# IRVLUTD/handnet-pipeline

Hardware: AMD Instinct MI355X
Metric: end-to-end frames/sec (FCOS+A2J, 640x480) (higher is better)
Workload: dtype f16x3 (fp32 values split into fp16 hi+lo, 3 MFMAs, fp32 accumulate; fp32 I/O); 1 GPU; Full HandNet pipeline (FCOS -> crop -> A2J), 640x480 RGB-D (BASELINE config 4); batch_per_gpu=32, global_batch=32, frame=640x480 RGB-D, parallelism=frames sharded over 1 GPU(s), one all-gather of per-frame records per step, rccl_ranks=1, ipc_mode=HSA_ENABLE_IPC_MODE_LEGACY=0, hipgraph=False

## Files before the change

handnet-pipeline_amd/csrc/conv_stem_direct.hip:

```cpp
#include "hn_common.h"

namespace {

typedef float f32x4 __attribute__((ext_vector_type(4)));
typedef _Float16 f16x8 __attribute__((ext_vector_type(8)));
typedef __attribute__((address_space(3))) void lds_void;
typedef __attribute__((address_space(1))) const void gbl_void;

constexpr int kPR = 15, kPC = 17;
constexpr int kQR = 7, kQC = 8;
constexpr int kIR = 2 * (kPR - 1) + 7;
constexpr int kIP = (2 * (kPC - 1) + 8) / 2;
constexpr int kPlanePieces = kIR * kIP;
constexpr int kPatchPieces = ((2 * kPlanePieces + 255) / 256) * 256;
constexpr int kWPieces = 64 * 7 * 8;
constexpr int kCout = 64;
constexpr int kPitch = kCout + 4;

struct StemParams {
  const _Float16* x;
  const _Float16* w;
  const float* bias;
  _Float16* y;
  int n, hb, wb, oh, ow, poh, pow_, ty, tx;
  long plane;
  int terms;
  int* range_flag;
};

__global__ __launch_bounds__(256, 2) void conv_stem_pool_direct_kernel(const StemParams p) {
  extern __shared__ __attribute__((aligned(1024))) char smem[];
  _Float16* patch = reinterpret_cast<_Float16*>(smem);
  _Float16* wbank = reinterpret_cast<_Float16*>(smem + kPatchPieces * 16);
  const int tid = threadIdx.x, lane = tid & 63, wave = tid >> 6, lg = lane >> 4, px = lane & 15;
  int lid;
  {
    const int bid = blockIdx.x, nb = gridDim.x;
    const int q = nb >> 3, rr = nb & 7, xcd = bid & 7, loc = bid >> 3;
    lid = (xcd < rr ? xcd * (q + 1) : rr * (q + 1) + (xcd - rr) * q) + loc;
  }
  const int per_img = p.ty * p.tx;
  const int img = lid / per_img;
  const int rem = lid - img * per_img;
  const int pty = rem / p.tx, ptx = rem - pty * p.tx;
  const int oy0 = 2 * kQR * pty - 1, ox0 = 2 * kQC * ptx - 1;
  const int r0 = 2 * oy0, c0p = ox0;

  const int wave_base = __builtin_amdgcn_readfirstlane(wave) * 64;
#pragma unroll
  for (int rnd = 0; rnd < kPatchPieces / 256; ++rnd) {
    const int q = rnd * 256 + tid;
    int pl = q >= kPlanePieces ? 1 : 0;
    int k = q - pl * kPlanePieces;
    if (k >= kPlanePieces) { pl = 1; k = kPlanePieces - 1; }
    const int row = k / kIP, pc = k - row * kIP;
    int sr = r0 + row, sc = c0p + pc;
    sr = sr < 0 ? 0 : (sr < p.hb ? sr : p.hb - 1);
    sc = sc < 0 ? 0 : (sc < (p.wb >> 1) ? sc : (p.wb >> 1) - 1);
    const _Float16* src = p.x + pl * p.plane + (((long)img * p.hb + sr) * p.wb + sc * 2) * 4;
    __builtin_amdgcn_global_load_lds((gbl_void*)src, (lds_void*)(smem + (rnd * 256 + wave_base) * 16), 16, 0, 0);
  }
#pragma unroll
  for (int rnd = 0; rnd < kWPieces / 256; ++rnd) {
    const _Float16* src = p.w + (long)(rnd * 256 + tid) * 8;
    __builtin_amdgcn_global_load_lds((gbl_void*)src, (lds_void*)(reinterpret_cast<char*>(wbank) + (rnd * 256 + wave_base) * 16), 16, 0,
                                     0);
  }

  int a_off[4];
  bool ok[4];
#pragma unroll
  for (int i = 0; i < 4; ++i) {
    int row = wave * 64 + i * 16 + px;
    ok[i] = row < kPR * kPC;
    row = ok[i] ? row : kPR * kPC - 1;
    const int pr = row / kPC, pc = row - pr * kPC;
    const int oy = oy0 + pr, ox = ox0 + pc;
    ok[i] = ok[i] && (unsigned)oy < (unsigned)p.oh && (unsigned)ox < (unsigned)p.ow;
    a_off[i] = ((2 * pr) * kIP + pc + lg) * 16;
  }
  const int b_off = (px * 7) * 128 + lg * 16;

  f32x4 acc[4][4];
#pragma unroll
  for (int i = 0; i < 4; ++i)
#pragma unroll
    for (int j = 0; j < 4; ++j) acc[i][j] = f32x4{0.f, 0.f, 0.f, 0.f};

  asm volatile("s_waitcnt vmcnt(0)" ::: "memory");
  __syncthreads();

  const char* pa = reinterpret_cast<const char*>(patch);
  const char* pb = reinterpret_cast<const char*>(wbank);
#pragma unroll 1
  for (int ky = 0; ky < 7; ++ky) {
    f16x8 ah[4], al[4], bh[4], bl[4];
#pragma unroll
    for (int i = 0; i < 4; ++i) {
      ah[i] = *reinterpret_cast<const f16x8*>(pa + a_off[i] + ky * (kIP * 16));
      al[i] = *reinterpret_cast<const f16x8*>(pa + a_off[i] + ky * (kIP * 16) + kPlanePieces * 16);
    }
#pragma unroll
    for (int j = 0; j < 4; ++j) {
      bh[j] = *reinterpret_cast<const f16x8*>(pb + b_off + j * (16 * 7 * 128) + ky * 128);
      bl[j] = *reinterpret_cast<const f16x8*>(pb + b_off + j * (16 * 7 * 128) + ky * 128 + 64);
    }
    if (p.terms == 3) {
#pragma unroll
      for (int i = 0; i < 4; ++i)
#pragma unroll
        for (int j = 0; j < 4; ++j) acc[i][j] = __builtin_amdgcn_mfma_f32_16x16x32_f16(bh[j], al[i], acc[i][j], 0, 0, 0);
#pragma unroll
      for (int i = 0; i < 4; ++i)
#pragma unroll
        for (int j = 0; j < 4; ++j) acc[i][j] = __builtin_amdgcn_mfma_f32_16x16x32_f16(bl[j], ah[i], acc[i][j], 0, 0, 0);
    }
#pragma unroll
    for (int i = 0; i < 4; ++i)
#pragma unroll
      for (int j = 0; j < 4; ++j) acc[i][j] = __builtin_amdgcn_mfma_f32_16x16x32_f16(bh[j], ah[i], acc[i][j], 0, 0, 0);
  }

  __syncthreads();
  float* fp = reinterpret_cast<float*>(smem);
  const int nsub = (lg & 1) * 16 + (lg >> 1) * 8;
#pragma unroll
  for (int i = 0; i < 4; ++i) {
    const int row = wave * 64 + i * 16 + px;
#pragma unroll
    for (int jp = 0; jp < 2; ++jp) {
      f32x4 x = acc[i][2 * jp], y = acc[i][2 * jp + 1];
#pragma unroll
      for (int r = 0; r < 4; ++r) {
        const auto s = __builtin_amdgcn_permlane16_swap(__float_as_uint(x[r]), __float_as_uint(y[r]), false, false);
        x[r] = __uint_as_float(s[0]);
        y[r] = __uint_as_float(s[1]);
      }
      const int n = jp * 32 + nsub;
      const f32x4 b0 = *reinterpret_cast<const f32x4*>(p.bias + n), b1 = *reinterpret_cast<const f32x4*>(p.bias + n + 4);
#pragma unroll
      for (int e = 0; e < 4; ++e) {
        x[e] = ok[i] ? hn::relu(x[e] + b0[e]) : 0.f;
        y[e] = ok[i] ? hn::relu(y[e] + b1[e]) : 0.f;
      }
      *reinterpret_cast<f32x4*>(fp + row * kPitch + n) = x;
      *reinterpret_cast<f32x4*>(fp + row * kPitch + n + 4) = y;
    }
  }
  __syncthreads();
  for (int item = tid; item < kQR * kQC * (kCout / 8); item += 256) {
    const int c8 = item & (kCout / 8 - 1), pp = item / (kCout / 8);
    const int pr = pp / kQC, pc = pp - pr * kQC;
    const int gy = kQR * pty + pr, gx = kQC * ptx + pc;
    if (gy >= p.poh || gx >= p.pow_) continue;
    f32x4 m0 = {0.f, 0.f, 0.f, 0.f}, m1 = m0;
#pragma unroll
    for (int dy = 0; dy < 3; ++dy)
#pragma unroll
      for (int dx = 0; dx < 3; ++dx) {
        const float* src = fp + ((2 * pr + dy) * kPC + 2 * pc + dx) * kPitch + c8 * 8;
        const f32x4 a = *reinterpret_cast<const f32x4*>(src), b = *reinterpret_cast<const f32x4*>(src + 4);
#pragma unroll
        for (int e = 0; e < 4; ++e) {
          m0[e] = hn::max_nan(m0[e], a[e]);
          m1[e] = hn::max_nan(m1[e], b[e]);
        }
      }
    f16x8 hi, lo;
    if (p.range_flag) {
      float mg = 0.f;
#pragma unroll
      for (int e = 0; e < 4; ++e) mg = hn::max_nan(mg, hn::range_mag(m0[e], m1[e]));
      if (!(mg <= 65504.f)) *p.range_flag = 1;
    }
#pragma unroll
    for (int e = 0; e < 4; ++e) {
      const _Float16 h0 = (_Float16)m0[e], h1 = (_Float16)m1[e];
      hi[e] = h0;
      hi[4 + e] = h1;
      lo[e] = (_Float16)(m0[e] - (float)h0);
      lo[4 + e] = (_Float16)(m1[e] - (float)h1);
    }
    _Float16* dst = p.y + (((long)img * p.poh + gy) * p.pow_ + gx) * (2 * kCout) + (c8 >> 2) * 64 + (c8 & 3) * 8;
    *reinterpret_cast<f16x8*>(dst) = hi;
    *reinterpret_cast<f16x8*>(dst + 32) = lo;
  }
}

}

namespace hn {

int stem_pool_direct(const void* x16, int n, int ph, int pw, const void* w16, const float* bias, void* y, int terms, hipStream_t st) {
  const int hb = ph + 6, wb = pw + 6;
  StemParams p;
  p.x = (const _Float16*)x16; p.w = (const _Float16*)w16; p.bias = bias; p.y = (_Float16*)y;
  p.n = n; p.hb = hb; p.wb = wb;
  p.oh = (hb - 7) / 2 + 1; p.ow = (wb - 7) / 2 + 1;
  p.poh = (p.oh + 2 - 3) / 2 + 1; p.pow_ = (p.ow + 2 - 3) / 2 + 1;
  p.ty = hn::cdiv(p.poh, kQR); p.tx = hn::cdiv(p.pow_, kQC);
  p.plane = (long)n * hb * wb * 4;
  p.terms = terms == 1 ? 1 : 3;
  p.range_flag = hn::range_flag_ptr();
  HN_CHECK_ARG(wb % 2 == 0 && (uintptr_t)x16 % 16 == 0 && (uintptr_t)w16 % 16 == 0 && (uintptr_t)y % 16 == 0 &&
                   (uintptr_t)bias % 16 == 0, "stem image rows / tensors must be 16-byte aligned");
  HN_CHECK_ARG((int64_t)n * p.ty * p.tx < (int64_t)1 << 31, "too many patches");
  constexpr int LDS_BYTES = kPatchPieces * 16 + kWPieces * 16;
  static_assert(LDS_BYTES <= 80 * 1024 && 256 * kPitch * 4 <= LDS_BYTES, "two workgroups per CU; the pooling patch reuses the space");
  static bool attr_set[64] = {};
  int dev = 0;
  HN_CHECK_HIP(hipGetDevice(&dev));
  if (dev < 0 || dev >= 64 || !attr_set[dev]) {
    HN_CHECK_HIP(hipFuncSetAttribute((const void*)conv_stem_pool_direct_kernel, hipFuncAttributeMaxDynamicSharedMemorySize, LDS_BYTES));
    if (dev >= 0 && dev < 64) attr_set[dev] = true;
  }
  hipLaunchKernelGGL(conv_stem_pool_direct_kernel, dim3(n * p.ty * p.tx), dim3(256), LDS_BYTES, st, p);
  HN_CHECK_LAUNCH("conv_stem_pool_direct_kernel");
  return HN_OK;
}

}
```

Measured before the change: 1167 frames/s.

## Make stem conv persistent and pool per 16-channel column tile

After: 1169 frames/s (median of 4 runs). About the same (+0.1%).

```diff
diff --git a/handnet-pipeline_amd/csrc/conv_stem_direct.hip b/handnet-pipeline_amd/csrc/conv_stem_direct.hip
--- a/handnet-pipeline_amd/csrc/conv_stem_direct.hip
+++ b/handnet-pipeline_amd/csrc/conv_stem_direct.hip
@@ -4,6 +4,7 @@
 
 typedef float f32x4 __attribute__((ext_vector_type(4)));
 typedef _Float16 f16x8 __attribute__((ext_vector_type(8)));
+typedef _Float16 f16x4 __attribute__((ext_vector_type(4)));
 typedef __attribute__((address_space(3))) void lds_void;
 typedef __attribute__((address_space(1))) const void gbl_void;
 
@@ -15,7 +16,7 @@
 constexpr int kPatchPieces = ((2 * kPlanePieces + 255) / 256) * 256;
 constexpr int kWPieces = 64 * 7 * 8;
 constexpr int kCout = 64;
-constexpr int kPitch = kCout + 4;
+constexpr int kPitch = 16 + 4;
 
 struct StemParams {
   const _Float16* x;
@@ -28,162 +29,153 @@
   int* range_flag;
 };
 
+__device__ __forceinline__ int xcd_remap(int v, int total) {
+  const int q = total >> 3, rr = total & 7, xcd = v & 7, loc = v >> 3;
+  return (xcd < rr ? xcd * (q + 1) : rr * (q + 1) + (xcd - rr) * q) + loc;
+}
+
 __global__ __launch_bounds__(256, 2) void conv_stem_pool_direct_kernel(const StemParams p) {
   extern __shared__ __attribute__((aligned(1024))) char smem[];
   _Float16* patch = reinterpret_cast<_Float16*>(smem);
   _Float16* wbank = reinterpret_cast<_Float16*>(smem + kPatchPieces * 16);
   const int tid = threadIdx.x, lane = tid & 63, wave = tid >> 6, lg = lane >> 4, px = lane & 15;
-  int lid;
-  {
-    const int bid = blockIdx.x, nb = gridDim.x;
-    const int q = nb >> 3, rr = nb & 7, xcd = bid & 7, loc = bid >> 3;
-    lid = (xcd < rr ? xcd * (q + 1) : rr * (q + 1) + (xcd - rr) * q) + loc;
-  }
   const int per_img = p.ty * p.tx;
-  const int img = lid / per_img;
-  const int rem = lid - img * per_img;
-  const int pty = rem / p.tx, ptx = rem - pty * p.tx;
-  const int oy0 = 2 * kQR * pty - 1, ox0 = 2 * kQC * ptx - 1;
-  const int r0 = 2 * oy0, c0p = ox0;
-
+  const int total = p.n * per_img;
   const int wave_base = __builtin_amdgcn_readfirstlane(wave) * 64;
-#pragma unroll
-  for (int rnd = 0; rnd < kPatchPieces / 256; ++rnd) {
-    const int q = rnd * 256 + tid;
-    int pl = q >= kPlanePieces ? 1 : 0;
-    int k = q - pl * kPlanePieces;
-    if (k >= kPlanePieces) { pl = 1; k = kPlanePieces - 1; }
-    const int row = k / kIP, pc = k - row * kIP;
-    int sr = r0 + row, sc = c0p + pc;
-    sr = sr < 0 ? 0 : (sr < p.hb ? sr : p.hb - 1);
-    sc = sc < 0 ? 0 : (sc < (p.wb >> 1) ? sc : (p.wb >> 1) - 1);
-    const _Float16* src = p.x + pl * p.plane + (((long)img * p.hb + sr) * p.wb + sc * 2) * 4;
-    __builtin_amdgcn_global_load_lds((gbl_void*)src, (lds_void*)(smem + (rnd * 256 + wave_base) * 16), 16, 0, 0);
-  }
+
 #pragma unroll
   for (int rnd = 0; rnd < kWPieces / 256; ++rnd) {
     const _Float16* src = p.w + (long)(rnd * 256 + tid) * 8;
     __builtin_amdgcn_global_load_lds((gbl_void*)src, (lds_void*)(reinterpret_cast<char*>(wbank) + (rnd * 256 + wave_base) * 16), 16, 0,
                                      0);
   }
-
-  int a_off[4];
-  bool ok[4];
-#pragma unroll
-  for (int i = 0; i < 4; ++i) {
-    int row = wave * 64 + i * 16 + px;
-    ok[i] = row < kPR * kPC;
-    row = ok[i] ? row : kPR * kPC - 1;
-    const int pr = row / kPC, pc = row - pr * kPC;
-    const int oy = oy0 + pr, ox = ox0 + pc;
-    ok[i] = ok[i] && (unsigned)oy < (unsigned)p.oh && (unsigned)ox < (unsigned)p.ow;
-    a_off[i] = ((2 * pr) * kIP + pc + lg) * 16;
-  }
   const int b_off = (px * 7) * 128 + lg * 16;
-
-  f32x4 acc[4][4];
-#pragma unroll
-  for (int i = 0; i < 4; ++i)
-#pragma unroll
-    for (int j = 0; j < 4; ++j) acc[i][j] = f32x4{0.f, 0.f, 0.f, 0.f};
-
-  asm volatile("s_waitcnt vmcnt(0)" ::: "memory");
-  __syncthreads();
-
-  const char* pa = reinterpret_cast<const char*>(patch);
-  const char* pb = reinterpret_cast<const char*>(wbank);
+  f32x4 bj[4];
+#pragma unroll
+  for (int j = 0; j < 4; ++j) bj[j] = *reinterpret_cast<const f32x4*>(p.bias + 16 * j + 4 * lg);
+
 #pragma unroll 1
-  for (int ky = 0; ky < 7; ++ky) {
-    f16x8 ah[4], al[4], bh[4], bl[4];
+  for (int v = blockIdx.x; v < total; v += gridDim.x) {
+    const int lid = xcd_remap(v, total);
+    const int img = lid / per_img;
+    const int rem = lid - img * per_img;
+    const int pty = rem / p.tx, ptx = rem - pty * p.tx;
+    const int oy0 = 2 * kQR * pty - 1, ox0 = 2 * kQC * ptx - 1;
+    const int r0 = 2 * oy0, c0p = ox0;
+
+#pragma unroll
+    for (int rnd = 0; rnd < kPatchPieces / 256; ++rnd) {
+      const int q = rnd * 256 + tid;
+      int pl = q >= kPlanePieces ? 1 : 0;
+      int k = q - pl * kPlanePieces;
+      if (k >= kPlanePieces) { pl = 1; k = kPlanePieces - 1; }
+      const int row = k / kIP, pc = k - row * kIP;
+      int sr = r0 + row, sc = c0p + pc;
+      sr = sr < 0 ? 0 : (sr < p.hb ? sr : p.hb - 1);
+      sc = sc < 0 ? 0 : (sc < (p.wb >> 1) ? sc : (p.wb >> 1) - 1);
+      const _Float16* src = p.x + pl * p.plane + (((long)img * p.hb + sr) * p.wb + sc * 2) * 4;
+      __builtin_amdgcn_global_load_lds((gbl_void*)src, (lds_void*)(smem + (rnd * 256 + wave_base) * 16), 16, 0, 0);
+    }
+
+    int a_off[4];
+    bool ok[4];
 #pragma unroll
     for (int i = 0; i < 4; ++i) {
-      ah[i] = *reinterpret_cast<const f16x8*>(pa + a_off[i] + ky * (kIP * 16));
-      al[i] = *reinterpret_cast<const f16x8*>(pa + a_off[i] + ky * (kIP * 16) + kPlanePieces * 16);
-    }
+      int row = wave * 64 + i * 16 + px;
+      ok[i] = row < kPR * kPC;
+      row = ok[i] ? row : kPR * kPC - 1;
+      const int pr = row / kPC, pc = row - pr * kPC;
+      const int oy = oy0 + pr, ox = ox0 + pc;
+      ok[i] = ok[i] && (unsigned)oy < (unsigned)p.oh && (unsigned)ox < (unsigned)p.ow;
+      a_off[i] = ((2 * pr) * kIP + pc + lg) * 16;
+    }
+
+    f32x4 acc[4][4];
+#pragma unroll
+    for (int i = 0; i < 4; ++i)
+#pragma unroll
+      for (int j = 0; j < 4; ++j) acc[i][j] = f32x4{0.f, 0.f, 0.f, 0.f};
+
+    asm volatile("s_waitcnt vmcnt(0)" ::: "memory");
+    __syncthreads();
+
+    const char* pa = reinterpret_cast<const char*>(patch);
+    const char* pb = reinterpret_cast<const char*>(wbank);
+#pragma unroll 1
+    for (int ky = 0; ky < 7; ++ky) {
+      f16x8 ah[4], al[4], bh[4], bl[4];
+#pragma unroll
+      for (int i = 0; i < 4; ++i) {
+        ah[i] = *reinterpret_cast<const f16x8*>(pa + a_off[i] + ky * (kIP * 16));
+        al[i] = *reinterpret_cast<const f16x8*>(pa + a_off[i] + ky * (kIP * 16) + kPlanePieces * 16);
+      }
+#pragma unroll
+      for (int j = 0; j < 4; ++j) {
+        bh[j] = *reinterpret_cast<const f16x8*>(pb + b_off + j * (16 * 7 * 128) + ky * 128);
+        bl[j] = *reinterpret_cast<const f16x8*>(pb + b_off + j * (16 * 7 * 128) + ky * 128 + 64);
+      }
+      if (p.terms == 3) {
+#pragma unroll
+        for (int i = 0; i < 4; ++i)
+#pragma unroll
+          for (int j = 0; j < 4; ++j) acc[i][j] = __builtin_amdgcn_mfma_f32_16x16x32_f16(bh[j], al[i], acc[i][j], 0, 0, 0);
+#pragma unroll
+        for (int i = 0; i < 4; ++i)
+#pragma unroll
+          for (int j = 0; j < 4; ++j) acc[i][j] = __builtin_amdgcn_mfma_f32_16x16x32_f16(bl[j], ah[i], acc[i][j], 0, 0, 0);
+      }
+#pragma unroll
+      for (int i = 0; i < 4; ++i)
+#pragma unroll
+        for (int j = 0; j < 4; ++j) acc[i][j] = __builtin_amdgcn_mfma_f32_16x16x32_f16(bh[j], ah[i], acc[i][j], 0, 0, 0);
+    }
+
+    float* fp = reinterpret_cast<float*>(smem);
 #pragma unroll
     for (int j = 0; j < 4; ++j) {
-      bh[j] = *reinterpret_cast<const f16x8*>(pb + b_off + j * (16 * 7 * 128) + ky * 128);
-      bl[j] = *reinterpret_cast<const f16x8*>(pb + b_off + j * (16 * 7 * 128) + ky * 128 + 64);
-    }
-    if (p.terms == 3) {
-#pragma unroll
-      for (int i = 0; i < 4; ++i)
-#pragma unroll
-        for (int j = 0; j < 4; ++j) acc[i][j] = __builtin_amdgcn_mfma_f32_16x16x32_f16(bh[j], al[i], acc[i][j], 0, 0, 0);
-#pragma unroll
-      for (int i = 0; i < 4; ++i)
-#pragma unroll
-        for (int j = 0; j < 4; ++j) acc[i][j] = __builtin_amdgcn_mfma_f32_16x16x32_f16(bl[j], ah[i], acc[i][j], 0, 0, 0);
-    }
-#pragma unroll
-    for (int i = 0; i < 4; ++i)
-#pragma unroll
-      for (int j = 0; j < 4; ++j) acc[i][j] = __builtin_amdgcn_mfma_f32_16x16x32_f16(bh[j], ah[i], acc[i][j], 0, 0, 0);
-  }
-
-  __syncthreads();
-  float* fp = reinterpret_cast<float*>(smem);
-  const int nsub = (lg & 1) * 16 + (lg >> 1) * 8;
-#pragma unroll
-  for (int i = 0; i < 4; ++i) {
-    const int row = wave * 64 + i * 16 + px;
-#pragma unroll
-    for (int jp = 0; jp < 2; ++jp) {
-      f32x4 x = acc[i][2 * jp], y = acc[i][2 * jp + 1];
-#pragma unroll
-      for (int r = 0; r < 4; ++r) {
-        const auto s = __builtin_amdgcn_permlane16_swap(__float_as_uint(x[r]), __float_as_uint(y[r]), false, false);
-        x[r] = __uint_as_float(s[0]);
-        y[r] = __uint_as_float(s[1]);
-      }
-      const int n = jp * 32 + nsub;
-      const f32x4 b0 = *reinterpret_cast<const f32x4*>(p.bias + n), b1 = *reinterpret_cast<const f32x4*>(p.bias + n + 4);
-#pragma unroll
-      for (int e = 0; e < 4; ++e) {
-        x[e] = ok[i] ? hn::relu(x[e] + b0[e]) : 0.f;
-        y[e] = ok[i] ? hn::relu(y[e] + b1[e]) : 0.f;
-      }
-      *reinterpret_cast<f32x4*>(fp + row * kPitch + n) = x;
-      *reinterpret_cast<f32x4*>(fp + row * kPitch + n + 4) = y;
-    }
-  }
-  __syncthreads();
-  for (int item = tid; item < kQR * kQC * (kCout / 8); item += 256) {
-    const int c8 = item & (kCout / 8 - 1), pp = item / (kCout / 8);
-    const int pr = pp / kQC, pc = pp - pr * kQC;
-    const int gy = kQR * pty + pr, gx = kQC * ptx + pc;
-    if (gy >= p.poh || gx >= p.pow_) continue;
-    f32x4 m0 = {0.f, 0.f, 0.f, 0.f}, m1 = m0;
-#pragma unroll
-    for (int dy = 0; dy < 3; ++dy)
-#pragma unroll
-      for (int dx = 0; dx < 3; ++dx) {
-        const float* src = fp + ((2 * pr + dy) * kPC + 2 * pc + dx) * kPitch + c8 * 8;
-        const f32x4 a = *reinterpret_cast<const f32x4*>(src), b = *reinterpret_cast<const f32x4*>(src + 4);
-#pragma unroll
-        for (int e = 0; e < 4; ++e) {
-          m0[e] = hn::max_nan(m0[e], a[e]);
-          m1[e] = hn::max_nan(m1[e], b[e]);
+      __syncthreads();
+#pragma unroll
+      for (int i = 0; i < 4; ++i) {
+        const int row = wave * 64 + i * 16 + px;
+        f32x4 x;
+#pragma unroll
+        for (int e = 0; e < 4; ++e) x[e] = ok[i] ? hn::relu(acc[i][j][e] + bj[j][e]) : 0.f;
+        *reinterpret_cast<f32x4*>(fp + row * kPitch + 4 * lg) = x;
+      }
+      __syncthreads();
+      if (tid < kQR * kQC * 4) {
+        const int c4 = tid & 3, pp = tid >> 2;
+        const int pr = pp / kQC, pc = pp - pr * kQC;
+        const int gy = kQR * pty + pr, gx = kQC * ptx + pc;
+        if (gy < p.poh && gx < p.pow_) {
+          f32x4 m = {0.f, 0.f, 0.f, 0.f};
+#pragma unroll
+          for (int dy = 0; dy < 3; ++dy)
+#pragma unroll
+            for (int dx = 0; dx < 3; ++dx) {
+              const f32x4 a = *reinterpret_cast<const f32x4*>(fp + ((2 * pr + dy) * kPC + 2 * pc + dx) * kPitch + c4 * 4);
+#pragma unroll
+              for (int e = 0; e < 4; ++e) m[e] = hn::max_nan(m[e], a[e]);
+            }
+          if (p.range_flag) {
+            const float mg = hn::max_nan(hn::range_mag(m[0], m[1]), hn::range_mag(m[2], m[3]));
+            if (!(mg <= 65504.f)) *p.range_flag = 1;
+          }
+          f16x4 hi, lo;
+#pragma unroll
+          for (int e = 0; e < 4; ++e) {
+            const _Float16 h = (_Float16)m[e];
+            hi[e] = h;
+            lo[e] = (_Float16)(m[e] - (float)h);
+          }
+          const int c = 16 * j + 4 * c4;
+          _Float16* dst = p.y + (((long)img * p.poh + gy) * p.pow_ + gx) * (2 * kCout) + (c >> 5) * 64 + (c & 31);
+          *reinterpret_cast<f16x4*>(dst) = hi;
+          *reinterpret_cast<f16x4*>(dst + 32) = lo;
         }
       }
-    f16x8 hi, lo;
-    if (p.range_flag) {
-      float mg = 0.f;
-#pragma unroll
-      for (int e = 0; e < 4; ++e) mg = hn::max_nan(mg, hn::range_mag(m0[e], m1[e]));
-      if (!(mg <= 65504.f)) *p.range_flag = 1;
-    }
-#pragma unroll
-    for (int e = 0; e < 4; ++e) {
-      const _Float16 h0 = (_Float16)m0[e], h1 = (_Float16)m1[e];
-      hi[e] = h0;
-      hi[4 + e] = h1;
-      lo[e] = (_Float16)(m0[e] - (float)h0);
-      lo[4 + e] = (_Float16)(m1[e] - (float)h1);
-    }
-    _Float16* dst = p.y + (((long)img * p.poh + gy) * p.pow_ + gx) * (2 * kCout) + (c8 >> 2) * 64 + (c8 & 3) * 8;
-    *reinterpret_cast<f16x8*>(dst) = hi;
-    *reinterpret_cast<f16x8*>(dst + 32) = lo;
+    }
+    __syncthreads();
   }
 }
 
@@ -206,15 +198,21 @@
                    (uintptr_t)bias % 16 == 0, "stem image rows / tensors must be 16-byte aligned");
   HN_CHECK_ARG((int64_t)n * p.ty * p.tx < (int64_t)1 << 31, "too many patches");
   constexpr int LDS_BYTES = kPatchPieces * 16 + kWPieces * 16;
-  static_assert(LDS_BYTES <= 80 * 1024 && 256 * kPitch * 4 <= LDS_BYTES, "two workgroups per CU; the pooling patch reuses the space");
-  static bool attr_set[64] = {};
+  static_assert(LDS_BYTES <= 80 * 1024 && 256 * kPitch * 4 <= kPatchPieces * 16,
+                "two workgroups per CU; the pooling patch of a column tile reuses the image patch's space");
+  static int cus[64] = {};
   int dev = 0;
   HN_CHECK_HIP(hipGetDevice(&dev));
-  if (dev < 0 || dev >= 64 || !attr_set[dev]) {
+  HN_CHECK_ARG(dev >= 0 && dev < 64, "device index out of range");
+  if (!cus[dev]) {
+    int c = 0;
+    HN_CHECK_HIP(hipDeviceGetAttribute(&c, hipDeviceAttributeMultiprocessorCount, dev));
     HN_CHECK_HIP(hipFuncSetAttribute((const void*)conv_stem_pool_direct_kernel, hipFuncAttributeMaxDynamicSharedMemorySize, LDS_BYTES));
-    if (dev >= 0 && dev < 64) attr_set[dev] = true;
+    cus[dev] = c > 0 ? c : 256;
   }
-  hipLaunchKernelGGL(conv_stem_pool_direct_kernel, dim3(n * p.ty * p.tx), dim3(256), LDS_BYTES, st, p);
+  const int patches = n * p.ty * p.tx;
+  const int grid = patches < 2 * cus[dev] ? patches : 2 * cus[dev];
+  hipLaunchKernelGGL(conv_stem_pool_direct_kernel, dim3(grid), dim3(256), LDS_BYTES, st, p);
   HN_CHECK_LAUNCH("conv_stem_pool_direct_kernel");
   return HN_OK;
 }
```
